# siddC/nbmf_mm

Hardware: AMD Instinct MI355X
Metric: MM-iterations/sec (higher is better)
Workload: dtype f64

## Files before the change

include/nbmf_hip.h:

```cpp
#ifndef NBMF_HIP_H
#define NBMF_HIP_H

#include <stdint.h>

#ifdef __cplusplus
extern "C" {
#endif

#define NBMF_OK 0
#define NBMF_ERR_ARG (-1)
#define NBMF_ERR_HIP (-2)
#define NBMF_ERR_RANGE (-3)
#define NBMF_ERR_STATE (-4)
#define NBMF_ERR_COMM (-5)

#define NBMF_MASK_NONE 0
#define NBMF_MASK_F64 1
#define NBMF_MASK_U8 2

#define NBMF_PROJ_NORMALIZE 0
#define NBMF_PROJ_DUCHI 1

#define NBMF_FLAG_BINARY_PATH 1

// ... 34 lines not shown
#define NBMF_STORAGE_F64_WEIGHTS 2
int nbmf_set_storage(nbmf_ctx* ctx, int storage);

int nbmf_get_n_obs(nbmf_ctx* ctx, double* n_obs);

int nbmf_set_factors(nbmf_ctx* ctx, const double* W_kxm, const double* H_kxn);
int nbmf_get_factors(nbmf_ctx* ctx, double* W_kxm, double* H_kxn);

int nbmf_run(nbmf_ctx* ctx, int max_iter, double tol, double* losses, int* n_iter);

int nbmf_run_batch(nbmf_ctx* ctx, int n_problems, const double* alpha, const double* beta, const double* W0, const double* H0,
                   int max_iter, double tol, double* losses, int* n_iter, double* W_out, double* H_out);
int nbmf_batch_stats(nbmf_ctx* ctx, int* launches, int* problems);
int nbmf_sweep_info(nbmf_ctx* ctx, int* h_chunks, int* h_blocks_per_chunk, int* w_chunks, int* w_blocks_per_chunk);
int nbmf_variant_stats(long long* full_w_launches, long long* ragged_k_launches, long long* loss_assembly_recoveries);

typedef void (*nbmf_progress_fn)(void* user, int first, int count, const double* losses);
int nbmf_set_progress(nbmf_ctx* ctx, nbmf_progress_fn fn, void* user, int every);

int nbmf_small_stats(nbmf_ctx* ctx, int* runs, int* aborted);

int nbmf_engine_stats(long long* persistent_served, long long* persistent_aborted, long long* launches_served);

int nbmf_w_only_steps(nbmf_ctx* ctx, int n_steps);

int nbmf_loss(nbmf_ctx* ctx, double* loss);

int nbmf_loglik(nbmf_ctx* ctx, int clip_theta, double* loglik);

int nbmf_loglik_strict(nbmf_ctx* ctx, double* loglik);
// ... 44 lines not shown
```

nbmf_mm_amd/_hip.py:

```python
from __future__ import annotations

import ctypes
import os
from ctypes import POINTER, byref, c_char_p, c_double, c_int, c_int64, c_void_p

import numpy as np

_HERE = os.path.dirname(os.path.abspath(__file__))

NBMF_OK = 0
NBMF_ERR_ARG = -1
NBMF_ERR_HIP = -2
NBMF_ERR_RANGE = -3
NBMF_ERR_STATE = -4
NBMF_ERR_COMM = -5

MASK_NONE, MASK_F64, MASK_U8 = 0, 1, 2
PROJ_NORMALIZE, PROJ_DUCHI = 0, 1
FLAG_BINARY_PATH = 1
STORAGE = {"auto": 0, "f64": 1, "f64w": 2}
MAX_K = 512
PEER_HANDLE_BYTES = 192

SYMBOLS = [
    "nbmf_abi_version", "nbmf_last_error", "nbmf_device_count", "nbmf_create", "nbmf_destroy",
    "nbmf_set_hyper", "nbmf_upload", "nbmf_upload_csr", "nbmf_generate", "nbmf_get_n_obs", "nbmf_set_factors", "nbmf_get_factors",
    "nbmf_run", "nbmf_w_only_steps", "nbmf_loss", "nbmf_loglik", "nbmf_loglik_strict", "nbmf_comm_unique_id", "nbmf_comm_init",
    "nbmf_comm_init_host", "nbmf_peer_export", "nbmf_comm_init_peer", "nbmf_comm_detach",
    "nbmf_timing_enable", "nbmf_timing_get", "nbmf_synchronize", "nbmf_selftest_unary",
    "nbmf_set_progress", "nbmf_device_synchronize", "nbmf_small_stats", "nbmf_generate_slice", "nbmf_set_storage",
    "nbmf_set_exchange_panels", "nbmf_set_peer_timeout_ms", "nbmf_run_batch", "nbmf_batch_stats", "nbmf_sweep_info",
    "nbmf_upload_v", "nbmf_selftest_mfma_peak", "nbmf_engine_stats", "nbmf_source_hash", "nbmf_comm_info", "nbmf_cancel", "nbmf_variant_stats", "nbmf_device_bus_id",
]
DATA_F64, DATA_U8, DATA_F32 = 0, 1, 2


HOST_ALLREDUCE_FN = ctypes.CFUNCTYPE(c_int, c_void_p, POINTER(c_double), c_int64)
PROGRESS_FN = ctypes.CFUNCTYPE(None, c_void_p, c_int, c_int, POINTER(c_double))


class NBMFHipError(RuntimeError):
    """A libnbmf_hip call failed (HIP error, missing GPU, bad state)."""


def library_path() -> str:
    return os.environ.get("NBMF_HIP_LIBRARY", os.path.join(_HERE, "libnbmf_hip.so"))

# ... 70 lines not shown
    lib.nbmf_upload.argtypes = [c_void_p, c_void_p, c_int64, c_int, c_void_p, c_int, c_int64, POINTER(c_int)]
    lib.nbmf_upload_v.argtypes = [c_void_p, c_void_p, c_int, c_int64, c_int, c_void_p, c_int, c_int64, POINTER(c_int)]
    lib.nbmf_selftest_mfma_peak.argtypes = [c_int, c_double, dp, dp, dp]
    lib.nbmf_engine_stats.argtypes = [POINTER(ctypes.c_longlong), POINTER(ctypes.c_longlong), POINTER(ctypes.c_longlong)]
    lib.nbmf_generate.argtypes = [c_void_p, ctypes.c_uint64, c_double, c_double]
    lib.nbmf_generate_slice.argtypes = [c_void_p, ctypes.c_uint64, c_double, c_double, c_int64, c_int64, c_int64]
    lib.nbmf_set_storage.argtypes = [c_void_p, c_int]
    lib.nbmf_get_n_obs.argtypes = [c_void_p, dp]
    lib.nbmf_set_factors.argtypes = [c_void_p, c_void_p, c_void_p]
    lib.nbmf_get_factors.argtypes = [c_void_p, c_void_p, c_void_p]
    lib.nbmf_run.argtypes = [c_void_p, c_int, c_double, c_void_p, POINTER(c_int)]
    lib.nbmf_run_batch.argtypes = [c_void_p, c_int, c_void_p, c_void_p, c_void_p, c_void_p, c_int, c_double, c_void_p, c_void_p,
                                   c_void_p, c_void_p]
    lib.nbmf_batch_stats.argtypes = [c_void_p, POINTER(c_int), POINTER(c_int)]
    lib.nbmf_sweep_info.argtypes = [c_void_p, POINTER(c_int), POINTER(c_int), POINTER(c_int), POINTER(c_int)]
    lib.nbmf_w_only_steps.argtypes = [c_void_p, c_int]
    lib.nbmf_loss.argtypes = [c_void_p, dp]
    lib.nbmf_loglik.argtypes = [c_void_p, c_int, dp]
    lib.nbmf_loglik_strict.argtypes = [c_void_p, dp]
    lib.nbmf_comm_unique_id.argtypes = [c_void_p]
    lib.nbmf_comm_init.argtypes = [c_void_p, c_void_p, c_int, c_int, c_int]
    lib.nbmf_comm_init_host.argtypes = [c_void_p, HOST_ALLREDUCE_FN, c_void_p, c_int, c_int, c_int]
    lib.nbmf_upload_csr.argtypes = [c_void_p, c_void_p, c_void_p, c_int64, c_int, c_void_p, c_void_p, c_int64, POINTER(c_int)]
    lib.nbmf_peer_export.argtypes = [c_void_p, c_int, c_void_p]
    lib.nbmf_comm_init_peer.argtypes = [c_void_p, c_void_p, c_int, c_int, c_int]
    lib.nbmf_comm_detach.argtypes = [c_void_p]
    lib.nbmf_set_exchange_panels.argtypes = [c_void_p, c_int]
    lib.nbmf_set_peer_timeout_ms.argtypes = [c_void_p, c_double]
    lib.nbmf_timing_enable.argtypes = [c_void_p, c_int]
    lib.nbmf_timing_get.argtypes = [c_void_p, dp, POINTER(c_int), dp, POINTER(c_int)]
# ... 181 lines not shown
        ptr = lambda a: a.ctypes.data_as(c_void_p)
        _check(self._lib.nbmf_run_batch(self._h, int(P), ptr(alphas), ptr(betas), ptr(W0), ptr(H0), int(max_iter), float(tol),
                                        ptr(losses), ptr(n_iter), ptr(W), ptr(H)))
        return [losses[p, :n_iter[p]].copy() for p in range(P)], n_iter, W, H

    def batch_stats(self):
        a, b = c_int(0), c_int(0)
        _check(self._lib.nbmf_batch_stats(self._h, byref(a), byref(b)))
        return a.value, b.value

    def sweep_info(self):
        v = [c_int(0) for _ in range(4)]
        _check(self._lib.nbmf_sweep_info(self._h, *[byref(x) for x in v]))
        return dict(zip(("h_chunks", "h_blocks", "w_chunks", "w_blocks"), (x.value for x in v)))

    def w_only_steps(self, n_steps):
        _check(self._lib.nbmf_w_only_steps(self._h, int(n_steps)))

    def loss(self):
        v = c_double(0)
        _check(self._lib.nbmf_loss(self._h, byref(v)))
        return v.value

    def loglik(self, clip_theta=False):
        v = c_double(0)
        _check(self._lib.nbmf_loglik(self._h, int(bool(clip_theta)), byref(v)))
        return v.value

    def loglik_strict(self):
        v = c_double(0)
# ... 136 lines not shown
```

nbmf_mm_amd/csrc/nbmf_hip.hip:

```cpp

#include <hip/hip_runtime.h>
#include <hip/hip_ext.h>

#include <dlfcn.h>
#include <unistd.h>
#include <algorithm>
#include <atomic>
#include <cmath>
#include <cstdarg>
#include <cstdint>
#include <cstdio>
#include <cstdlib>
#include <cstring>
#include <chrono>
#include <condition_variable>
#include <map>
#include <mutex>
#include <string>
#include <type_traits>
#include <vector>

#include "../../include/nbmf_hip.h"

#ifndef NBMF_NO_MFMA
// ... 205 lines not shown
  int data_kind = -1;
  int storage = NBMF_STORAGE_AUTO;
  void *dataA = nullptr, *dataB = nullptr, *maskA = nullptr, *maskB = nullptr;
  unsigned long long *bitsA = nullptr, *bitsB = nullptr;
  double n_obs = 0, n_obs_global = 0;
  double* rowcnt = nullptr;
  double *Wn = nullptr, *WT = nullptr, *WG = nullptr, *Hn = nullptr, *HT = nullptr, *HG = nullptr;
  bool have_factors = false;
  bool padB_ones = false;
  bool w_free = false;
  bool factors_in_range = false;
  int chunksH = 0, CH_H = 0, chunksW = 0, CH_W = 0;
  int *cstartH = nullptr, *cstartW = nullptr;
  double *slabH = nullptr, *slabW = nullptr, *Pbuf = nullptr, *lossbuf = nullptr, *prior = nullptr, *scal = nullptr;
  double* lossfin = nullptr;
  int n_prior_blocks = 0;
  int* flags = nullptr;
  double* losses_d = nullptr;
  int losses_cap = 0;
  double* stage = nullptr;
  size_t stage_bytes = 0;
  unsigned long long* stats = nullptr;
  double alpha = 1.2, beta = 1.2, eps = 1e-8;
  int projection = NBMF_PROJ_NORMALIZE;
  void* comm = nullptr;
  nbmf_host_allreduce_fn host_reduce = nullptr;
  void* host_reduce_user = nullptr;
  double* host_buf = nullptr;
  size_t host_buf_count = 0;
  int nranks = 1, rank = 0;
// ... 413 lines not shown
      if (cnt[w]) fprintf(stderr, " slot %d: %.1f us (%d)", w, dur[w] / cnt[w] * 0.01, cnt[w]);
    fprintf(stderr, "\n");
    std::sort(exits.begin(), exits.end());
    const double us = 0.01;
    fprintf(stderr, "[nbmf] pass<K=%d,data=%d,mode=%d> %zu workgroups: span %.1f us | entries spread over %.1f us | exits: first %.1f, median %.1f, "
                    "last %.1f us before the end | per workgroup: prologue %.2f, loop %.2f, epilogue %.2f us (loss block %.2f, slab stores %.2f) | shader clock in the loops %.3f GHz\n", K, data, mode, live,
            (double)(t_last - t_first) * us, (double)(last_entry - t_first) * us, (double)(t_last - first_exit) * us,
            ((double)t_last - exits[exits.size() / 2]) * us, 0.0, pro / live * us, loop / live * us, epi / live * us, epi_loss / live * us,
            epi_slab / live * us, loop > 0 ? loop_clk / loop * 0.1 : 0.0);
  }
  return hipSuccess;
}

template <int KB, int DATA, int MODE, int TH, bool TINY, bool RAG = false, bool FULL = false>
hipError_t launch_pass_tt(const PassArgs& a_, int chunks, hipStream_t st) {
  if (FULL) g_full_w_launches.fetch_add(1, std::memory_order_relaxed);
  if (RAG) g_ragged_launches.fetch_add(1, std::memory_order_relaxed);
  dim3 grid(a_.Cb / WG_WAVES, chunks);
  constexpr int lds_bytes = pass_lds_bytes(KB, DATA, MODE);
  if (lds_bytes > 65536) {
    hipError_t e = hipFuncSetAttribute((const void*)pass_kernel<KB, DATA, MODE, TH, TINY, RAG, FULL>, hipFuncAttributeMaxDynamicSharedMemorySize, lds_bytes);
    if (e != hipSuccess) return e;
  }
  PassArgs a = a_;
  if (DATA != DATA_BIN && MODE != MODE_W && MODE != MODE_T && pass_log_bits(KB) == 10) {
    hipError_t e = log_table_device(&a.ltab_g);
    if (e != hipSuccess) return e;
  }
  static std::atomic<long> trace_count{0};
  if (MODE != MODE_T && pass_trace_due(trace_count))
// ... 457 lines not shown

int enqueue_h_update_from(nbmf_ctx* c, const double* src, bool slabs, hipStream_t st) {
  const size_t per = (size_t)std::min(c->KP, SLICE_K) * c->nA;
  const int chunks = slabs ? c->chunksH : 1;
  for (int sl = 0; sl < c->KS; ++sl) {
    launch_h_update(c, src + (size_t)sl * chunks * per, chunks, slabs ? per : 0, 0, c->nA, sl, slabs ? pform_inv12(c) : 0.0, st);
    HIPCHK(hipGetLastError());
  }
  c->prior_src = c->prior;
  c->n_prior_src = c->n_prior_blocks;
  return NBMF_OK;
}
int enqueue_h_update(nbmf_ctx* c) { return enqueue_h_update_from(c, c->slabH, true, c->stream); }

template <int GROUPS>
int launch_w_update(nbmf_ctx* c, const double* q, int chunks, double n_div, int projection) {
  const size_t lds_bytes = sizeof(double) * ((size_t)c->KP + 2) * WU_COLS;
  if (lds_bytes > 65536)
    HIPCHK(hipFuncSetAttribute((const void*)w_update_kernel<GROUPS>, hipFuncAttributeMaxDynamicSharedMemorySize, (int)lds_bytes));
  hipLaunchKernelGGL(w_update_kernel<GROUPS>, dim3((unsigned)(c->mA / WU_COLS)), dim3(WU_COLS * GROUPS), lds_bytes, c->stream, q,
                     chunks, c->Wn, c->WT, c->WG, c->k, c->KP, std::min(c->KP, SLICE_K), (long long)c->m, (long long)c->mA, n_div,
                     c->rowcnt, projection, c->flags);
  HIPCHK(hipGetLastError());
  return NBMF_OK;
}
int enqueue_w_update(nbmf_ctx* c, const double* q, int chunks, double n_div, int projection) {
  return c->mA / WU_COLS <= 4LL * c->cus ? launch_w_update<32>(c, q, chunks, n_div, projection)
                                        : launch_w_update<8>(c, q, chunks, n_div, projection);
}

int enqueue_reduce_h_all(nbmf_ctx* c, double* dst, hipStream_t st) {
  const size_t per = (size_t)std::min(c->KP, SLICE_K) * c->nA, tot = (size_t)c->KP * c->nA;
  for (int sl = 0; sl < c->KS; ++sl) {
    launch_reduce_h(c, sl, 0, c->nA, dst + sl * per, c->nA, sl == 0 ? dst + 2 * tot : (double*)nullptr, st);
    HIPCHK(hipGetLastError());
  }
  return NBMF_OK;
}

int enqueue_w_step(nbmf_ctx* c, int projection);

int enqueue_iteration_rows_peer(nbmf_ctx* c, int it, double tol) {
  const size_t per = (size_t)c->KP * c->nA;
  {
    EvScope ev(c, 0, true, c->KS == 1);
    if (c->KS > 1) {
      if (int rc = enqueue_a_sweeps_sliced(c, true, 0, 0)) return rc;
    } else {
      HIPCHK(launch_pass<MODE_H>(c->KB, c->data_kind, h_pass_args(c), c->chunksH, c->stream));
    }
  }
  double* X = c->arena;
  const unsigned long long hs = ++c->hseq;
  const int slots_per_panel = PEER_H_WGS * c->pv.nranks;
  const long long offPR_now = c->offPR + (long long)(hs & 1) * 2 * 2 * PEER_H_WGS * PEER_MAX_RANKS;
// ... 122 lines not shown
  {
    EvScope ev(c, 1);
    HIPCHK(launch_pass<MODE_W>(c->KB, c->data_kind, w, first, s0));
    if (c->npanel == 2) {
      if (two_streams) {
        HIPCHK(hipStreamWaitEvent(s0, c->ev1, 0));
      } else {
        w.chunk0 = first;
        HIPCHK(launch_pass<MODE_W>(c->KB, c->data_kind, w, c->chunksW - first, s0));
      }
    }
  }
  return enqueue_w_update(c, c->slabW, c->chunksW, (double)c->n, c->projection);
}

int enqueue_w_step(nbmf_ctx* c, int projection) {
  if (c->KS > 1) {
    {
      EvScope ev(c, 1);
      if (int rc = enqueue_theta(c, 1)) return rc;
      for (int step = 0; step < c->KS; ++step) {
        const int sl = step == 0 ? c->KS - 1 : step - 1;
        PassArgs w = w_pass_args(c);
        at_slice(c, w, 1, sl);
        w.theta = c->theta;
        if (step == 0)
          HIPCHK((launch_pass_slice<MODE_W, 2>(c->data_kind, w, c->chunksW, c->stream)));
        else
          HIPCHK((launch_pass_slice<MODE_W, 1>(c->data_kind, w, c->chunksW, c->stream)));
      }
    }
    if (is_sharded(c) && c->shard_axis == 1) {
      const long long per = (long long)SLICE_K * c->mA;
      for (int sl = 0; sl < c->KS; ++sl) {
        hipLaunchKernelGGL(reduce_w_kernel, dim3((unsigned)((per + 255) / 256)), dim3(256), 0, c->stream,
                           (const double*)(c->slabW + (size_t)sl * c->chunksW * per), c->Qbuf + sl * per, c->chunksW, per, c->flags);
        HIPCHK(hipGetLastError());
      }
      if (int rc = all_reduce_inplace(c, c->Qbuf, (size_t)c->KP * c->mA)) return rc;
      return enqueue_w_update(c, c->Qbuf, 1, c->n_div_global, projection);
    }
    return enqueue_w_update(c, c->slabW, c->chunksW, (double)c->n, projection);
  }
  PassArgs a = w_pass_args(c);
  {
    EvScope ev(c, 1, true, true);
    HIPCHK(launch_pass<MODE_W>(c->KB, c->data_kind, a, c->chunksW, c->stream));
  }
  const double* q = c->slabW;
  int chunks = c->chunksW;
  double n_div = (double)c->n;
  if (is_sharded(c) && c->shard_axis == 1) {
    const long long per = (long long)c->KP * c->mA;
    hipLaunchKernelGGL(reduce_w_kernel, dim3((unsigned)((per + 255) / 256)), dim3(256), 0, c->stream,
                       (const double*)c->slabW, c->Qbuf, c->chunksW, per, c->flags);
    HIPCHK(hipGetLastError());
    if (int rc = all_reduce_inplace(c, c->Qbuf, (size_t)per)) return rc;
    q = c->Qbuf;
    chunks = 1;
    n_div = c->n_div_global;
  }
  return enqueue_w_update(c, q, chunks, n_div, projection);
}
// ... 556 lines not shown
  for (int** p : {&c->cstartH, &c->cstartW}) {
    if (*p) HIPCHK(dfree(*p));
    *p = nullptr;
  }
  HIPCHK(dmalloc(&c->cstartH, sizeof(int) * bH.size()));
  HIPCHK(dmalloc(&c->cstartW, sizeof(int) * bW.size()));
  HIPCHK(hipMemcpy(c->cstartH, bH.data(), sizeof(int) * bH.size(), hipMemcpyHostToDevice));
  HIPCHK(hipMemcpy(c->cstartW, bW.data(), sizeof(int) * bW.size(), hipMemcpyHostToDevice));
  if (env_set("NBMF_DEBUG"))
    fprintf(stderr, "[nbmf] K_pad=%d path=%d: H-pass %d x %d workgroups (chunk %d blocks, %d slots), W-pass %d x %d (chunk %d, %d slots)\n",
            c->KP, c->data_kind, (int)(c->nA / 64), c->chunksH, c->CH_H, slotsH, (int)(c->mA / 64), c->chunksW, c->CH_W, slotsW);
  for (double** p : {&c->slabH, &c->slabW, &c->lossbuf, &c->lossfin}) {
    if (*p) HIPCHK(dfree(*p));
    *p = nullptr;
  }
  for (unsigned long long** p : {&c->bitsA, &c->bitsB}) {
    if (*p) HIPCHK(dfree(*p));
    *p = nullptr;
  }
  if (c->data_kind == DATA_BIN) {
    const long long n_tiles = (long long)(c->mA / 16) * (c->nA / 16);
    HIPCHK(dmalloc(&c->bitsA, sizeof(unsigned long long) * 8 * (size_t)n_tiles + PASS_SLACK));
    HIPCHK(dmalloc(&c->bitsB, sizeof(unsigned long long) * 8 * (size_t)n_tiles + PASS_SLACK));
    for (int image = 0; image < 2; ++image) {
      hipLaunchKernelGGL(mask_build_kernel, dim3((unsigned)((n_tiles + 3) / 4)), dim3(256), 0, c->stream,
                         (const uint32_t*)(image == 0 ? c->dataA : c->dataB), image == 0 ? c->bitsA : c->bitsB, n_tiles);
      HIPCHK(hipGetLastError());
    }
  }
  const size_t fw = (size_t)c->KP * c->mA * sizeof(double), fh = (size_t)c->KP * c->nA * sizeof(double);
  HIPCHK(dmalloc(&c->slabH, 2 * (size_t)c->chunksH * fh));
  HIPCHK(dmalloc(&c->slabW, (size_t)c->chunksW * fw));
  const size_t n_slots = (size_t)c->chunksH * (c->nA / 16 / WG_WAVES);
  HIPCHK(dmalloc(&c->lossbuf, sizeof(double) * n_slots));
  HIPCHK(dmalloc(&c->lossfin, sizeof(double) * n_slots));
  if (int rc = fill_ll_empty(c)) return rc;
  return NBMF_OK;
}

void comm_release(nbmf_ctx* c, bool recount = false) {
  if (recount && is_sharded(c) && c->shard_axis == 1 && c->data_kind >= 0) {
    hipLaunchKernelGGL(rowcount_kernel, dim3((unsigned)((c->m + 255) / 256)), dim3(256), 0, c->stream, c->dataB, c->maskB,
                       c->data_kind, (long long)(c->nA / 16), (long long)c->m, (long long)c->n, c->rowcnt);
    hipStreamSynchronize(c->stream);
  }
  if (c->comm && g_rccl.CommDestroy) g_rccl.CommDestroy(c->comm);
  c->comm = nullptr;
// ... 155 lines not shown
  ctx_guard.p = nullptr;
  *out = c;
  return NBMF_OK;
}

int nbmf_destroy(nbmf_ctx* c) {
  if (!c) return NBMF_OK;
  hipSetDevice(c->device);
  if (c->stream) hipStreamSynchronize(c->stream);
  comm_release(c);
  if (c->host_buf) hipHostFree(c->host_buf);
  arena_release((ArenaSlot*)c->arena_slot.p);
  void* ptrs[] = {c->dataA, c->dataB, c->maskA, c->maskB, c->rowcnt, c->Wn, c->WT, c->WG, c->Hn, c->HT, c->HG,
                  c->slabH, c->slabW, c->Pbuf, c->lossbuf, c->lossfin, c->prior, c->scal, c->flags, c->losses_d, c->stage, c->stats,
                  c->sbuf, c->Qbuf, c->cstartH, c->cstartW, c->theta, c->small.slab, c->small_batch.slab, c->small_batch.table,
                  c->small_batch.io, c->bitsA, c->bitsB};
  for (void* p : ptrs)
    if (p) dfree(p);
  for (hipEvent_t e : c->ev) hipEventDestroy(e);
  for (hipEvent_t e : {c->evH, c->evF, c->ev1})
    if (e) hipEventDestroy(e);
  if (c->stream2) {
    hipStreamSynchronize(c->stream2);
    hipStreamDestroy(c->stream2);
  }
  if (c->stream) stream_release(c->device, c->stream);
  delete c;
  return NBMF_OK;
}

int nbmf_set_hyper(nbmf_ctx* c, double alpha, double beta, double eps, int projection) {
// ... 379 lines not shown
  const int batch = progress ? c->progress_every : (tol > 0.0) ? 8 : max_iter;
  int reported = 0;
  std::vector<double> fresh;
  auto report = [&](int n_final) -> int {
    if (!progress || n_final <= reported) return NBMF_OK;
    fresh.resize((size_t)(n_final - reported));
    HIPCHK(hipMemcpy(fresh.data(), c->losses_d + reported, sizeof(double) * fresh.size(), hipMemcpyDeviceToHost));
    c->progress(c->progress_user, reported, n_final - reported, fresh.data());
    reported = n_final;
    return NBMF_OK;
  };
  int host_done = 0;
  int it = 0;
  const bool use_graph = env_set("NBMF_USE_GRAPH") && !is_sharded(c) && !c->timing && !progress && max_iter >= 8;
  bool fused_fin = fin_fusable(c) && !use_graph;
  int recoveries = 0;
  int fl[8];
  auto settle = [&](bool at_end, bool* resume) -> int {
    *resume = false;
    HIPCHK(hipMemcpyAsync(fl, c->flags, sizeof fl, hipMemcpyDeviceToHost, c->stream));
    HIPCHK(hipStreamSynchronize(c->stream));
    if (c->timing) timing_collect(c);
    if (int rc = peer_check(c)) return rc;
    if (!fl[6] || !fused_fin || recoveries >= 4 || (at_end && c->cancelled.load(std::memory_order_relaxed))) return NBMF_OK;
    ++recoveries;
    g_loss_assembly_recoveries.fetch_add(1, std::memory_order_relaxed);
    if (env_set("NBMF_DEBUG")) fprintf(stderr, "[nbmf] loss %d could not be assembled inside its sweep within the bound: resuming with separate launches\n", fl[1]);
    fused_fin = false;
    if (int rc = fill_ll_empty(c)) return rc;
    HIPCHK(hipMemsetAsync(c->flags, 0, sizeof(int), c->stream));
    HIPCHK(hipMemsetAsync(c->flags + 6, 0, sizeof(int), c->stream));
    it = fl[1] + 1;
    host_done = 0;
    *resume = true;
    return NBMF_OK;
  };
  hipGraph_t graph = nullptr;
  hipGraphExec_t gexec = nullptr;
// ... 26 lines not shown
          HIPCHK(hipGraphLaunch(gexec, c->stream));
          continue;
        }
        if (is_sharded(c) && c->shard_axis == 0) {
          if (int rc = enqueue_iteration_rows(c, it, tol)) return rc;
          continue;
        }
        if (fused_fin) {
          if (int rc = enqueue_a_sweep(c, true, 0, 0, it - 1, tol)) return rc;
        } else {
          if (int rc = enqueue_a_sweep(c, true)) return rc;
          if (it > 0)
            if (int rc = enqueue_finalize(c, it - 1, tol)) return rc;
        }
        if (int rc = enqueue_h_update(c)) return rc;
        if (int rc = enqueue_w_step(c, c->projection)) return rc;
      }
      if ((tol > 0.0 || progress) && it < max_iter) {
        bool resume = false;
        if (int rc = settle(false, &resume)) return rc;
        if (!resume) {
          host_done = fl[0];
          if (int rc = report(fl[1])) return rc;
        }
      }
      continue;
    }
    if (!host_done) {
      if (fused_fin) {
        if (int rc = enqueue_a_sweep(c, false, 0, 0, max_iter - 1, tol)) return rc;
      } else {
// ... 57 lines not shown

int nbmf_sweep_info(nbmf_ctx* c, int* h_chunks, int* h_blocks, int* w_chunks, int* w_blocks) {
  if (!c) return fail(NBMF_ERR_ARG, "null context");
  if (!c->cstartH) return fail(NBMF_ERR_STATE, "no data on the device yet");
  if (h_chunks) *h_chunks = c->chunksH;
  if (h_blocks) *h_blocks = c->CH_H;
  if (w_chunks) *w_chunks = c->chunksW;
  if (w_blocks) *w_blocks = c->CH_W;
  return NBMF_OK;
}

int nbmf_variant_stats(long long* full_w_launches, long long* ragged_k_launches, long long* loss_assembly_recoveries) {
  if (full_w_launches) *full_w_launches = g_full_w_launches.load(std::memory_order_relaxed);
  if (ragged_k_launches) *ragged_k_launches = g_ragged_launches.load(std::memory_order_relaxed);
  if (loss_assembly_recoveries) *loss_assembly_recoveries = g_loss_assembly_recoveries.load(std::memory_order_relaxed);
  return NBMF_OK;
}

int nbmf_w_only_steps(nbmf_ctx* c, int n_steps) {
  if (int rc = ready(c)) return rc;
  if (n_steps < 0) return fail(NBMF_ERR_ARG, "n_steps must be >= 0");
  if (int rc = set_device(c)) return rc;
  HIPCHK(hipMemsetAsync(c->flags, 0, sizeof(int) * 8, c->stream));
  struct FreeW {
    nbmf_ctx* c;
    ~FreeW() { c->w_free = false; }
  } free_w{c};
  c->w_free = true;
  for (int s = 0; s < n_steps; ++s) {
    if (int rc = enqueue_w_step(c, NBMF_PROJ_NORMALIZE)) return rc;
// ... 449 lines not shown
```

nbmf_mm_amd/csrc/nbmf_pass_kernel.inc:

```

#define NBMF_DIV(y_, d_) ((y_) * rcp_nr(d_))
#define NBMF_DIV2(ya_, da_, yb_, db_, qa_, qb_) \
  {                                             \
    const double it_ = rcp_nr((da_) * (db_));   \
    qa_ = (ya_) * (it_ * (db_));                \
    qb_ = (yb_) * (it_ * (da_));                \
  }

#if NBMF_NO_MFMA
__device__ __forceinline__ d4 mfma_stub(double a, double b, d4 c) {
  __asm__ volatile("" : "+v"(c) : "v"(a), "v"(b));
  return c;
}
#define NBMF_MFMA(a_, b_, c_, x_, y_, z_) mfma_stub((a_), (b_), (c_))
#else
#define NBMF_MFMA(a_, b_, c_, x_, y_, z_) __builtin_amdgcn_mfma_f64_16x16x4f64((a_), (b_), (c_), (x_), (y_), (z_))
#endif

typedef __attribute__((address_space(3))) char lds_char;
typedef const __attribute__((address_space(1))) char glb_char;
typedef const __attribute__((address_space(1))) uint32_t glb_u32;
template <int PPW>
__device__ __forceinline__ void dma_run(glb_char* g, lds_char* l) {
  static_assert(PPW == 2 || PPW == 4, "2 KiB or 4 KiB per wave and image");
// ... 16 lines not shown
struct PassFin {
  int on;
  unsigned long long wait_ticks;
  int t;
  int n_ll, n_prior;
  double ll_pad, am1, bm1, n_obs, tol;
  const double* prior;
  double* losses;
  double* scal;
  int* flags;
};
template <bool SC1>
__device__ __forceinline__ void finalize_block(const double* ll_src, int n_ll, double ll_pad, const double* prior, int n_prior,
                                               double am1, double bm1, double n_obs, double* __restrict__ losses, int t,
                                               double tol, double* __restrict__ scal, int* __restrict__ flags, double (*sh)[4]);

struct PassArgs {
  const void* data;
  const void* mask;
  const double2* ltab_g;
  const double* LT;
  const double* LG;
  const double* RfT;
  double* out1;
  double* out2;
  double* lossbuf;
  const int* done;
  int Rb;
  int Cb;
  const int* chunk_start;
  int chunk0;
  long long C_alloc;
  double eps;
  int strict;
  int clip;
  double* theta;
  int accum;
  int tiny_eps;
  int ksteps, kblocks;
  int full;
  PassFin fin;
  unsigned long long* trace;
};

constexpr int pass_log_bits(int KB) { return KB == 8 ? 8 : 10; }
constexpr int pass_lds_bytes(int KB, int DATA, int MODE) {
  return (KB <= 4 ? STAGE_BYTES : 2 * STAGE_BYTES) + ((DATA != DATA_BIN && MODE != MODE_W && MODE != MODE_T) ? (16 << pass_log_bits(KB)) : 0);
}
constexpr int pass_wgs_per_cu(int KB, int DATA, int MODE) {
  if (KB == 8) return (MODE == MODE_H && DATA != DATA_BIN) ? 1 : 2;
  if (DATA != DATA_BIN && MODE == MODE_H) return 2;
  if (DATA == DATA_F64 && MODE == MODE_L && KB == 1) return 2;
  return 3;
}
template <int KB, int DATA, int MODE, int TH = 0, bool TINY = false, bool RAG = false, bool FULL = false>
__global__ __launch_bounds__(64 * WG_WAVES, pass_wgs_per_cu(KB, DATA, MODE)) void pass_kernel(PassArgs a) {
  static_assert(TH == 0 || MODE != MODE_T, "a Theta sweep does not read Theta");
  static_assert(!FULL || (MODE == MODE_W && DATA == DATA_BIN && TH == 0 && !TINY), "the two-state variant: W sweeps of the binary path's plain variant");
  static_assert(!TINY || MODE != MODE_T, "eps does not change the code of the Theta sweeps");
  static_assert(!RAG || (TH == 0 && !TINY && MODE != MODE_T && KB <= 4), "the ragged-K variant: one slice, plain variant, fused sweeps, up to the K = 64 layout");
  [[maybe_unused]] const int ksteps = a.ksteps, kblocks = a.kblocks;
  constexpr bool PRODUCTS = (MODE == MODE_H || MODE == MODE_W);
  constexpr int K = 16 * KB;
  constexpr int S = K / 4;
  constexpr int NB = (KB >= 4) ? 1 : 4 / KB;
  constexpr int BLK = K * 16;
  constexpr int STAGE_D = 2 * NB * BLK;
  constexpr int N2 = NB * BLK / 2;
  extern __shared__ __attribute__((aligned(16))) double lds[];
// ... 628 lines not shown
        __hip_atomic_store(a.lossbuf + (size_t)chunk * gridDim.x + bx, t, __ATOMIC_RELAXED, __HIP_MEMORY_SCOPE_AGENT);
    }
  }

  [[maybe_unused]] unsigned long long tr3 = 0, tr4 = 0;
  if (a.trace) tr3 = wall_clock64();
  const int q = lane >> 4, c = lane & 15;
  {
    if (MODE == MODE_W) {
      s2 += __shfl_xor(s2, 16, 64);
      s2 += __shfl_xor(s2, 32, 64);
    }
    [[maybe_unused]] const double inv12 = 1.0 / c12;
    double* o1 = a.out1 + (size_t)chunk * K * a.C_alloc + (size_t)cb * 16 + c;
    double* o2 = (MODE == MODE_H) ? a.out2 + (size_t)chunk * K * a.C_alloc + (size_t)cb * 16 + c : nullptr;
    if (PRODUCTS) {
#pragma unroll
      for (int kb = 0; kb < KB; ++kb) {
#pragma unroll
        for (int r = 0; r < 4; ++r) {
          const size_t k = 16 * kb + 4 * r + q;
          if (MODE == MODE_H) {
            o1[k * a.C_alloc] = acc1[kb][r];
            o2[k * a.C_alloc] = acc2[kb][r];
          } else {
            o1[k * a.C_alloc] = ZE_W ? __builtin_fma(s2, inv12, acc1[kb][r]) : acc1[kb][r] + s2;
          }
        }
      }
    }
// ... 58 lines not shown
```

nbmf_mm_amd/csrc/nbmf_update_kernels.inc:

```

__device__ __forceinline__ size_t t_index(long long k, long long x, int KS, long long lenA) {
  return (size_t)(k / KS) * KS * lenA + (size_t)((x >> 4) * KS + (k % KS)) * 16 + (x & 15);
}
__device__ __forceinline__ size_t g_index(long long k, long long x, int KS, long long lenA) {
  const long long kk = k % KS;
  return (size_t)(k / KS) * KS * lenA + (size_t)(x >> 4) * KS * 16 + (kk >> 4) * 256 + (x & 15) * 16 + (kk & 15);
}

__device__ __forceinline__ double ordered_sum256(const double* __restrict__ p, int n, int stride, double* sh4) {
  double s = 0.0;
  for (int j = threadIdx.x; j < n; j += 256) s += p[(size_t)j * stride];
  s = wave_sum(s);
  __syncthreads();
  if ((threadIdx.x & 63) == 0) sh4[threadIdx.x >> 6] = s;
  __syncthreads();
  return ((sh4[0] + sh4[1]) + sh4[2]) + sh4[3];
}

__global__ __launch_bounds__(256) void reduce_h_kernel(const double* __restrict__ slab1, const double* __restrict__ slab2,
                                                       int chunks, long long per , long long nA,
                                                       long long c0, long long wp, long long dst_ld, int KP,
                                                       double* __restrict__ dst1, double* __restrict__ dst2,
                                                       const double* __restrict__ lossbuf,
                                                       int n_loss, double ll_pad, double* __restrict__ ll_dst,
// ... 177 lines not shown
  if (flags[0]) return;
  if (t < 0) {
    const int armed = flags[3];
    __syncthreads();
    if (!armed) {
      if (threadIdx.x == 0) flags[3] = 1;
      return;
    }
    t = flags[2];
  }
  __shared__ double sh[3][4];
  finalize_block<false>(ll_src, n_ll, ll_pad, prior, n_prior, am1, bm1, n_obs, losses, t, tol, scal, flags, sh);
}

constexpr int WU_COLS = 32;
template <int WU_GROUPS>
__global__ __launch_bounds__(WU_COLS * WU_GROUPS) void w_update_kernel(const double* __restrict__ slab, int chunks, double* __restrict__ Wn,
                                                       double* __restrict__ WT, double* __restrict__ WG, int K, int KP,
                                                       int KS , long long m,
                                                       long long mA, double n_div,
                                                       const double* __restrict__ rowcnt, int projection,
                                                       const int* done) {
  extern __shared__ __attribute__((aligned(16))) double tile[];
  if (*done) return;
  const int c = threadIdx.x & (WU_COLS - 1), g = threadIdx.x / WU_COLS;
  const long long i = (long long)blockIdx.x * WU_COLS + c;
  const size_t per = (size_t)KS * mA;
  const bool live = i < m;
  double div = n_div;
  if (live && projection == NBMF_PROJ_DUCHI && rowcnt) div = fmax(rowcnt[i], 1.0);
  for (int k = g; k < K; k += WU_GROUPS) {
    double w = 0.0;
    if (live) {
      double qv = 0.0;
      const double* sk = slab + (size_t)(k / KS) * chunks * per + (size_t)(k % KS) * mA + i;
      for (int ch = 0; ch < chunks; ++ch) qv += sk[(size_t)ch * per];
      w = (Wn[(size_t)k * mA + i] * qv) / div;
    }
    tile[k * WU_COLS + c] = w;
  }
  __syncthreads();
  double* par = tile + (size_t)KP * WU_COLS;
  if (g == 0) {
    double sum = 0.0;
    for (int k = 0; k < K; ++k) sum += tile[k * WU_COLS + c];
    double tau = 0.0, scale = 1.0;
    if (projection == NBMF_PROJ_DUCHI) {
      tau = (sum - 1.0) / K;
      int cnt = K;
      for (int it = 0; it < K; ++it) {
        double s = 0.0;
        int c2 = 0;
        for (int k = 0; k < K; ++k) {
          const double v = tile[k * WU_COLS + c];
          if (v > tau) {
            s += v;
            ++c2;
          }
        }
        if (c2 == 0) break;
        const bool same = (c2 == cnt);
        tau = (s - 1.0) / c2;
        cnt = c2;
        if (same) break;
      }
    } else {
      scale = sum;
    }
    par[c] = scale;
    par[WU_COLS + c] = tau;
  }
  __syncthreads();
  const double scale = par[c], tau = par[WU_COLS + c];
  for (int k = g; k < KP; k += WU_GROUPS) {
    double w = 0.0;
    if (live && k < K) {
      const double v = tile[k * WU_COLS + c];
      w = (projection == NBMF_PROJ_DUCHI) ? fmax(v - tau, 0.0) : v / scale;
    }
    Wn[(size_t)k * mA + i] = w;
    WT[t_index(k, i, KS, mA)] = w;
    WG[g_index(k, i, KS, mA)] = w;
  }
}

__global__ void set_factor_kernel(const double* __restrict__ src, double* __restrict__ Fn, double* __restrict__ FT,
                                  double* __restrict__ FG, int K, int KP, int KS, long long len, long long lenA) {
  const long long idx = (long long)blockIdx.x * blockDim.x + threadIdx.x;
  if (idx >= (long long)KP * lenA) return;
  const long long k = idx / lenA, x = idx % lenA;
  const double v = (k < K && x < len) ? src[k * len + x] : 0.0;
  Fn[idx] = v;
  FT[t_index(k, x, KS, lenA)] = v;
  FG[g_index(k, x, KS, lenA)] = v;
}

__global__ void factor_range_kernel(const double* __restrict__ Wn, const double* __restrict__ Hn, int K, long long m,
// ... 29 lines not shown
```

Baseline: 202.8.

## Fuse W update into W pass epilogue with cross-chunk ticket handoff

When the W sweep has at most two chunks and no sharding, the pass kernel's epilogue now applies the multiplicative W update and projection directly. It uses an atomic ticket so the second chunk's workgroup waits for the first chunk's partial sums through the slab. This removes the separate w_update_kernel launch and its slab re-read per iteration. A bounded spin with a timeout flag falls back to separate launches, and the host resumes from the failing iteration. The cost is extra epilogue work, atomic handoff, and slab reset traffic.

After: 201.6. About the same (-0.6%).

```diff
diff --git a/include/nbmf_hip.h b/include/nbmf_hip.h
--- a/include/nbmf_hip.h
+++ b/include/nbmf_hip.h
@@ -72,6 +72,7 @@
 int nbmf_batch_stats(nbmf_ctx* ctx, int* launches, int* problems);
 int nbmf_sweep_info(nbmf_ctx* ctx, int* h_chunks, int* h_blocks_per_chunk, int* w_chunks, int* w_blocks_per_chunk);
 int nbmf_variant_stats(long long* full_w_launches, long long* ragged_k_launches, long long* loss_assembly_recoveries);
+int nbmf_fused_w_stats(nbmf_ctx* ctx, long long* fused_sweeps, long long* recoveries);
 
 typedef void (*nbmf_progress_fn)(void* user, int first, int count, const double* losses);
 int nbmf_set_progress(nbmf_ctx* ctx, nbmf_progress_fn fn, void* user, int every);
diff --git a/nbmf_mm_amd/_hip.py b/nbmf_mm_amd/_hip.py
--- a/nbmf_mm_amd/_hip.py
+++ b/nbmf_mm_amd/_hip.py
@@ -31,6 +31,7 @@
     "nbmf_set_progress", "nbmf_device_synchronize", "nbmf_small_stats", "nbmf_generate_slice", "nbmf_set_storage",
     "nbmf_set_exchange_panels", "nbmf_set_peer_timeout_ms", "nbmf_run_batch", "nbmf_batch_stats", "nbmf_sweep_info",
     "nbmf_upload_v", "nbmf_selftest_mfma_peak", "nbmf_engine_stats", "nbmf_source_hash", "nbmf_comm_info", "nbmf_cancel", "nbmf_variant_stats", "nbmf_device_bus_id",
+    "nbmf_fused_w_stats",
 ]
 DATA_F64, DATA_U8, DATA_F32 = 0, 1, 2
 
@@ -131,6 +132,7 @@
                                    c_void_p, c_void_p]
     lib.nbmf_batch_stats.argtypes = [c_void_p, POINTER(c_int), POINTER(c_int)]
     lib.nbmf_sweep_info.argtypes = [c_void_p, POINTER(c_int), POINTER(c_int), POINTER(c_int), POINTER(c_int)]
+    lib.nbmf_fused_w_stats.argtypes = [c_void_p, POINTER(ctypes.c_longlong), POINTER(ctypes.c_longlong)]
     lib.nbmf_w_only_steps.argtypes = [c_void_p, c_int]
     lib.nbmf_loss.argtypes = [c_void_p, dp]
     lib.nbmf_loglik.argtypes = [c_void_p, c_int, dp]
@@ -342,6 +344,11 @@
         _check(self._lib.nbmf_sweep_info(self._h, *[byref(x) for x in v]))
         return dict(zip(("h_chunks", "h_blocks", "w_chunks", "w_blocks"), (x.value for x in v)))
 
+    def fused_w_stats(self):
+        a, b = ctypes.c_longlong(0), ctypes.c_longlong(0)
+        _check(self._lib.nbmf_fused_w_stats(self._h, byref(a), byref(b)))
+        return a.value, b.value
+
     def w_only_steps(self, n_steps):
         _check(self._lib.nbmf_w_only_steps(self._h, int(n_steps)))
 
diff --git a/nbmf_mm_amd/csrc/nbmf_hip.hip b/nbmf_mm_amd/csrc/nbmf_hip.hip
--- a/nbmf_mm_amd/csrc/nbmf_hip.hip
+++ b/nbmf_mm_amd/csrc/nbmf_hip.hip
@@ -243,6 +243,8 @@
   int *cstartH = nullptr, *cstartW = nullptr;
   double *slabH = nullptr, *slabW = nullptr, *Pbuf = nullptr, *lossbuf = nullptr, *prior = nullptr, *scal = nullptr;
   double* lossfin = nullptr;
+  int* wfuse = nullptr;
+  long long fused_w_sweeps = 0, fused_w_recoveries = 0;
   int n_prior_blocks = 0;
   int* flags = nullptr;
   double* losses_d = nullptr;
@@ -686,6 +688,7 @@
 
 template <int KB, int DATA, int MODE, int TH, bool TINY, bool RAG = false, bool FULL = false>
 hipError_t launch_pass_tt(const PassArgs& a_, int chunks, hipStream_t st) {
+  if (a_.wup.on && !pass_has_wup(KB, MODE, TH, RAG)) return hipErrorInvalidValue;
   if (FULL) g_full_w_launches.fetch_add(1, std::memory_order_relaxed);
   if (RAG) g_ragged_launches.fetch_add(1, std::memory_order_relaxed);
   dim3 grid(a_.Cb / WG_WAVES, chunks);
@@ -1173,19 +1176,19 @@
 int enqueue_h_update(nbmf_ctx* c) { return enqueue_h_update_from(c, c->slabH, true, c->stream); }
 
 template <int GROUPS>
-int launch_w_update(nbmf_ctx* c, const double* q, int chunks, double n_div, int projection) {
+int launch_w_update(nbmf_ctx* c, const double* q, int chunks, double n_div, int projection, const int* applied, int epoch) {
   const size_t lds_bytes = sizeof(double) * ((size_t)c->KP + 2) * WU_COLS;
   if (lds_bytes > 65536)
     HIPCHK(hipFuncSetAttribute((const void*)w_update_kernel<GROUPS>, hipFuncAttributeMaxDynamicSharedMemorySize, (int)lds_bytes));
   hipLaunchKernelGGL(w_update_kernel<GROUPS>, dim3((unsigned)(c->mA / WU_COLS)), dim3(WU_COLS * GROUPS), lds_bytes, c->stream, q,
                      chunks, c->Wn, c->WT, c->WG, c->k, c->KP, std::min(c->KP, SLICE_K), (long long)c->m, (long long)c->mA, n_div,
-                     c->rowcnt, projection, c->flags);
+                     c->rowcnt, projection, c->flags, applied, epoch);
   HIPCHK(hipGetLastError());
   return NBMF_OK;
 }
-int enqueue_w_update(nbmf_ctx* c, const double* q, int chunks, double n_div, int projection) {
-  return c->mA / WU_COLS <= 4LL * c->cus ? launch_w_update<32>(c, q, chunks, n_div, projection)
-                                        : launch_w_update<8>(c, q, chunks, n_div, projection);
+int enqueue_w_update(nbmf_ctx* c, const double* q, int chunks, double n_div, int projection, const int* applied = nullptr, int epoch = 0) {
+  return c->mA / WU_COLS <= 4LL * c->cus ? launch_w_update<32>(c, q, chunks, n_div, projection, applied, epoch)
+                                        : launch_w_update<8>(c, q, chunks, n_div, projection, applied, epoch);
 }
 
 int enqueue_reduce_h_all(nbmf_ctx* c, double* dst, hipStream_t st) {
@@ -1197,7 +1200,7 @@
   return NBMF_OK;
 }
 
-int enqueue_w_step(nbmf_ctx* c, int projection);
+int enqueue_w_step(nbmf_ctx* c, int projection, int fuse_epoch = 0, int rest_of_epoch = 0);
 
 int enqueue_iteration_rows_peer(nbmf_ctx* c, int it, double tol) {
   const size_t per = (size_t)c->KP * c->nA;
@@ -1350,7 +1353,23 @@
   return enqueue_w_update(c, c->slabW, c->chunksW, (double)c->n, c->projection);
 }
 
-int enqueue_w_step(nbmf_ctx* c, int projection) {
+bool w_update_fusable(const nbmf_ctx* c) {
+  if (c->KB >= 4 && c->k < 16 * c->KB) return false;
+  if (c->mA >= (1LL << 26)) return false;
+  return !is_sharded(c) && c->KS == 1 && c->chunksW <= 2 && c->wfuse && !env_set("NBMF_NO_FUSED_W_UPDATE");
+}
+int* w_applied(const nbmf_ctx* c) { return c->wfuse + c->mA / 64; }
+int w_fuse_arm(nbmf_ctx* c) {
+  HIPCHK(hipMemsetAsync(c->wfuse, 0, sizeof(int) * (size_t)(c->mA / 64 + c->mA / 16), c->stream));
+  if (c->chunksW == 2) {
+    const size_t n = (size_t)c->chunksW * c->KP * c->mA;
+    hipLaunchKernelGGL(fill_u64_kernel, dim3((unsigned)((n + 255) / 256)), dim3(256), 0, c->stream, (unsigned long long*)c->slabW, n, LL_EMPTY);
+    HIPCHK(hipGetLastError());
+  }
+  return NBMF_OK;
+}
+
+int enqueue_w_step(nbmf_ctx* c, int projection, int fuse_epoch, int rest_of_epoch) {
   if (c->KS > 1) {
     {
       EvScope ev(c, 1);
@@ -1379,10 +1398,29 @@
     return enqueue_w_update(c, c->slabW, c->chunksW, (double)c->n, projection);
   }
   PassArgs a = w_pass_args(c);
+  if (fuse_epoch > 0) {
+    a.wup.on = 1;
+    a.wup.epoch = fuse_epoch;
+    a.wup.wait_ticks = env_int("NBMF_FUSED_W_FAULT", 0) == 2 ? 0ull : LL_WAIT_TICKS;
+    a.wup.projection = projection;
+    a.wup.K = c->k;
+    a.wup.m = c->m;
+    a.wup.n_div = (double)c->n;
+    a.wup.rowcnt = c->rowcnt;
+    a.wup.Wn = c->Wn;
+    a.wup.WT = c->WT;
+    a.wup.WG = c->WG;
+    a.wup.ticket = (unsigned*)c->wfuse;
+    a.wup.applied = w_applied(c);
+    a.wup.flags = c->flags;
+    ++c->fused_w_sweeps;
+  }
   {
     EvScope ev(c, 1, true, true);
     HIPCHK(launch_pass<MODE_W>(c->KB, c->data_kind, a, c->chunksW, c->stream));
   }
+  if (fuse_epoch > 0) return NBMF_OK;
+  if (rest_of_epoch > 0) return enqueue_w_update(c, c->slabW, c->chunksW, (double)c->n, projection, w_applied(c), rest_of_epoch);
   const double* q = c->slabW;
   int chunks = c->chunksW;
   double n_div = (double)c->n;
@@ -1969,6 +2007,8 @@
     if (*p) HIPCHK(dfree(*p));
     *p = nullptr;
   }
+  if (c->wfuse) HIPCHK(dfree(c->wfuse));
+  c->wfuse = nullptr;
   for (unsigned long long** p : {&c->bitsA, &c->bitsB}) {
     if (*p) HIPCHK(dfree(*p));
     *p = nullptr;
@@ -1986,6 +2026,7 @@
   const size_t fw = (size_t)c->KP * c->mA * sizeof(double), fh = (size_t)c->KP * c->nA * sizeof(double);
   HIPCHK(dmalloc(&c->slabH, 2 * (size_t)c->chunksH * fh));
   HIPCHK(dmalloc(&c->slabW, (size_t)c->chunksW * fw));
+  HIPCHK(dmalloc(&c->wfuse, sizeof(int) * (size_t)(c->mA / 64 + c->mA / 16)));
   const size_t n_slots = (size_t)c->chunksH * (c->nA / 16 / WG_WAVES);
   HIPCHK(dmalloc(&c->lossbuf, sizeof(double) * n_slots));
   HIPCHK(dmalloc(&c->lossfin, sizeof(double) * n_slots));
@@ -2171,7 +2212,7 @@
   void* ptrs[] = {c->dataA, c->dataB, c->maskA, c->maskB, c->rowcnt, c->Wn, c->WT, c->WG, c->Hn, c->HT, c->HG,
                   c->slabH, c->slabW, c->Pbuf, c->lossbuf, c->lossfin, c->prior, c->scal, c->flags, c->losses_d, c->stage, c->stats,
                   c->sbuf, c->Qbuf, c->cstartH, c->cstartW, c->theta, c->small.slab, c->small_batch.slab, c->small_batch.table,
-                  c->small_batch.io, c->bitsA, c->bitsB};
+                  c->small_batch.io, c->bitsA, c->bitsB, c->wfuse};
   for (void* p : ptrs)
     if (p) dfree(p);
   for (hipEvent_t e : c->ev) hipEventDestroy(e);
@@ -2581,6 +2622,9 @@
   int it = 0;
   const bool use_graph = env_set("NBMF_USE_GRAPH") && !is_sharded(c) && !c->timing && !progress && max_iter >= 8;
   bool fused_fin = fin_fusable(c) && !use_graph;
+  bool fused_w = w_update_fusable(c) && !use_graph;
+  if (fused_w)
+    if (int rc = w_fuse_arm(c)) return rc;
   int recoveries = 0;
   int fl[8];
   auto settle = [&](bool at_end, bool* resume) -> int {
@@ -2589,6 +2633,18 @@
     HIPCHK(hipStreamSynchronize(c->stream));
     if (c->timing) timing_collect(c);
     if (int rc = peer_check(c)) return rc;
+    if (fl[7] && fused_w && !(at_end && c->cancelled.load(std::memory_order_relaxed))) {
+      ++c->fused_w_recoveries;
+      if (env_set("NBMF_DEBUG")) fprintf(stderr, "[nbmf] the W sweep of iteration %d could not apply all of its update within the bound: resuming with separate launches\n", fl[7] - 1);
+      fused_w = false;
+      HIPCHK(hipMemsetAsync(c->flags, 0, sizeof(int), c->stream));
+      HIPCHK(hipMemsetAsync(c->flags + 7, 0, sizeof(int), c->stream));
+      if (int rc = enqueue_w_step(c, c->projection, 0, fl[7])) return rc;
+      it = fl[7];
+      host_done = 0;
+      *resume = true;
+      return NBMF_OK;
+    }
     if (!fl[6] || !fused_fin || recoveries >= 4 || (at_end && c->cancelled.load(std::memory_order_relaxed))) return NBMF_OK;
     ++recoveries;
     g_loss_assembly_recoveries.fetch_add(1, std::memory_order_relaxed);
@@ -2645,7 +2701,7 @@
             if (int rc = enqueue_finalize(c, it - 1, tol)) return rc;
         }
         if (int rc = enqueue_h_update(c)) return rc;
-        if (int rc = enqueue_w_step(c, c->projection)) return rc;
+        if (int rc = enqueue_w_step(c, c->projection, fused_w ? it + 1 : 0)) return rc;
       }
       if ((tol > 0.0 || progress) && it < max_iter) {
         bool resume = false;
@@ -2733,6 +2789,13 @@
   if (full_w_launches) *full_w_launches = g_full_w_launches.load(std::memory_order_relaxed);
   if (ragged_k_launches) *ragged_k_launches = g_ragged_launches.load(std::memory_order_relaxed);
   if (loss_assembly_recoveries) *loss_assembly_recoveries = g_loss_assembly_recoveries.load(std::memory_order_relaxed);
+  return NBMF_OK;
+}
+
+int nbmf_fused_w_stats(nbmf_ctx* c, long long* fused_sweeps, long long* recoveries) {
+  if (!c) return fail(NBMF_ERR_ARG, "null context");
+  if (fused_sweeps) *fused_sweeps = c->fused_w_sweeps;
+  if (recoveries) *recoveries = c->fused_w_recoveries;
   return NBMF_OK;
 }
 
diff --git a/nbmf_mm_amd/csrc/nbmf_pass_kernel.inc b/nbmf_mm_amd/csrc/nbmf_pass_kernel.inc
--- a/nbmf_mm_amd/csrc/nbmf_pass_kernel.inc
+++ b/nbmf_mm_amd/csrc/nbmf_pass_kernel.inc
@@ -54,6 +54,29 @@
 __device__ __forceinline__ void finalize_block(const double* ll_src, int n_ll, double ll_pad, const double* prior, int n_prior,
                                                double am1, double bm1, double n_obs, double* __restrict__ losses, int t,
                                                double tol, double* __restrict__ scal, int* __restrict__ flags, double (*sh)[4]);
+
+struct PassWup {
+  int on;
+  int epoch;
+  unsigned long long wait_ticks;
+  int projection, K;
+  long long m;
+  double n_div;
+  const double* rowcnt;
+  double *Wn, *WT, *WG;
+  unsigned* ticket;
+  int* applied;
+  int* flags;
+};
+__device__ __forceinline__ size_t t_index(long long k, long long x, int KS, long long lenA);
+__device__ __forceinline__ size_t g_index(long long k, long long x, int KS, long long lenA);
+__device__ __forceinline__ double wu_div(bool live, long long i, double n_div, const double* __restrict__ rowcnt, int projection);
+__device__ __forceinline__ double wu_times(double w, double qv);
+__device__ __forceinline__ double wu_over(double p, double div);
+__device__ __forceinline__ void wu_column(const double* tile, int stride, int K, int projection, double* scale_out, double* tau_out);
+__device__ __forceinline__ double wu_value(double v, double scale, double tau, int projection);
+__device__ __forceinline__ void wu_store(double* __restrict__ Wn, double* __restrict__ WT, double* __restrict__ WG, long long k,
+                                         long long i, int KS, long long mA, double w);
 
 struct PassArgs {
   const void* data;
@@ -80,6 +103,7 @@
   int ksteps, kblocks;
   int full;
   PassFin fin;
+  PassWup wup;
   unsigned long long* trace;
 };
 
@@ -93,6 +117,7 @@
   if (DATA == DATA_F64 && MODE == MODE_L && KB == 1) return 2;
   return 3;
 }
+constexpr bool pass_has_wup(int KB, int MODE, int TH, bool RAG) { return MODE == MODE_W && TH == 0 && !(RAG && KB >= 4); }
 template <int KB, int DATA, int MODE, int TH = 0, bool TINY = false, bool RAG = false, bool FULL = false>
 __global__ __launch_bounds__(64 * WG_WAVES, pass_wgs_per_cu(KB, DATA, MODE)) void pass_kernel(PassArgs a) {
   static_assert(TH == 0 || MODE != MODE_T, "a Theta sweep does not read Theta");
@@ -751,6 +776,111 @@
     [[maybe_unused]] const double inv12 = 1.0 / c12;
     double* o1 = a.out1 + (size_t)chunk * K * a.C_alloc + (size_t)cb * 16 + c;
     double* o2 = (MODE == MODE_H) ? a.out2 + (size_t)chunk * K * a.C_alloc + (size_t)cb * 16 + c : nullptr;
+    constexpr bool WUP = pass_has_wup(KB, MODE, TH, RAG);
+    if (WUP && a.wup.on) {
+      const unsigned long long rowB = (unsigned long long)a.C_alloc * 8ull;
+      unsigned lane_slab = (unsigned)q * (unsigned)rowB + (unsigned)c * 8u;
+      typedef __attribute__((address_space(1))) char glb_wchar;
+      typedef __attribute__((address_space(1))) unsigned long long glb_u64;
+#pragma unroll
+      for (int kb = 0; kb < KB; ++kb) {
+#pragma unroll
+        for (int r = 0; r < 4; ++r) acc1[kb][r] = 0.0 + (ZE_W ? __builtin_fma(s2, inv12, acc1[kb][r]) : acc1[kb][r] + s2);
+      }
+      bool apply = true;
+      if (gridDim.y == 2) {
+        volatile unsigned* tk = (volatile unsigned*)lds;
+        if (threadIdx.x == 0) *tk = __hip_atomic_fetch_add(a.wup.ticket + bx, 1u, __ATOMIC_RELAXED, __HIP_MEMORY_SCOPE_AGENT);
+        __syncthreads();
+        const bool second = __builtin_amdgcn_readfirstlane((int)(*tk & 1u)) != 0;
+        __syncthreads();
+        const int sc = second ? (chunk ^ 1) : chunk;
+        const unsigned long long sb = scalar64((unsigned long long)(a.out1 + (size_t)sc * K * a.C_alloc + (size_t)cb * 16));
+        if (!second) {
+#pragma unroll
+          for (int kb = 0; kb < KB; ++kb) {
+#pragma unroll
+            for (int r = 0; r < 4; ++r)
+              __hip_atomic_store((glb_u64*)((glb_wchar*)(sb + (unsigned long long)(16 * kb + 4 * r) * rowB) + lane_slab),
+                                 (unsigned long long)__double_as_longlong(acc1[kb][r]), __ATOMIC_RELAXED, __HIP_MEMORY_SCOPE_AGENT);
+          }
+          apply = false;
+        } else {
+          constexpr int GK = KB < 4 ? KB : 4;
+          const unsigned long long t0 = (unsigned long long)wall_clock64();
+#pragma unroll
+          for (int g0 = 0; g0 < KB; g0 += GK) {
+            d4 oth[GK];
+            for (;;) {
+              bool missing = false;
+              __asm__ volatile("" : "+v"(lane_slab));
+#pragma unroll
+              for (int kb = 0; kb < GK; ++kb) {
+#pragma unroll
+                for (int r = 0; r < 4; ++r) {
+                  const unsigned long long v = __hip_atomic_load((glb_u64*)((glb_wchar*)(sb + (unsigned long long)(16 * (g0 + kb) + 4 * r) * rowB) + lane_slab),
+                                                                 __ATOMIC_RELAXED, __HIP_MEMORY_SCOPE_AGENT);
+                  missing |= v == LL_EMPTY;
+                  oth[kb][r] = __longlong_as_double((long long)v);
+                }
+              }
+              if (__builtin_amdgcn_ballot_w64(missing) == 0ull) break;
+              if ((unsigned long long)wall_clock64() - t0 > a.wup.wait_ticks) {
+                apply = false;
+                break;
+              }
+              __builtin_amdgcn_s_sleep(8);
+            }
+            if (!apply) break;
+#pragma unroll
+            for (int kb = 0; kb < GK; ++kb) {
+#pragma unroll
+              for (int r = 0; r < 4; ++r) {
+                __hip_atomic_store((glb_u64*)((glb_wchar*)(sb + (unsigned long long)(16 * (g0 + kb) + 4 * r) * rowB) + lane_slab), LL_EMPTY,
+                                   __ATOMIC_RELAXED, __HIP_MEMORY_SCOPE_AGENT);
+                acc1[g0 + kb][r] = (chunk == 0) ? acc1[g0 + kb][r] + oth[kb][r] : (0.0 + oth[kb][r]) + acc1[g0 + kb][r];
+              }
+            }
+          }
+          if (!apply && lane == 0) {
+            a.wup.flags[0] = 1;
+            a.wup.flags[7] = a.wup.epoch;
+          }
+        }
+      }
+      if (apply) {
+        const long long i = (long long)cb * 16 + c;
+        const bool live = i < a.wup.m;
+        const int projection = a.wup.projection, Kr = a.wup.K;
+        const double div = wu_div(live, i, a.wup.n_div, a.wup.rowcnt, projection);
+        double* tile = lds + wave * (K * 16) + c;
+#pragma unroll
+        for (int kb = 0; kb < KB; ++kb) {
+#pragma unroll
+          for (int r = 0; r < 4; ++r) tile[(16 * kb + 4 * r + q) * 16] = acc1[kb][r];
+        }
+        {
+          double w[S];
+#pragma unroll
+          for (int s = 0; s < S; ++s) w[s] = a.RfT[((size_t)cb * S + s) * 64 + lane];
+#pragma unroll
+          for (int s = 0; s < S; ++s) tile[(4 * s + q) * 16] = wu_times(w[s], tile[(4 * s + q) * 16]);
+        }
+#pragma unroll 1
+        for (int k = q; k < K; k += 4) tile[k * 16] = live ? wu_over(tile[k * 16], div) : 0.0;
+        __builtin_amdgcn_fence(__ATOMIC_RELEASE, "wavefront");
+        __builtin_amdgcn_wave_barrier();
+        __builtin_amdgcn_fence(__ATOMIC_ACQUIRE, "wavefront");
+        double scale, tau;
+        wu_column(tile, 16, Kr, projection, &scale, &tau);
+#pragma unroll 1
+        for (int k = q; k < K; k += 4) {
+          const double w = (live && k < Kr) ? wu_value(tile[k * 16], scale, tau, projection) : 0.0;
+          wu_store(a.wup.Wn, a.wup.WT, a.wup.WG, k, i, K, a.C_alloc, w);
+        }
+        if (lane == 0) a.wup.applied[cb] = a.wup.epoch;
+      }
+    } else
     if (PRODUCTS) {
 #pragma unroll
       for (int kb = 0; kb < KB; ++kb) {
diff --git a/nbmf_mm_amd/csrc/nbmf_update_kernels.inc b/nbmf_mm_amd/csrc/nbmf_update_kernels.inc
--- a/nbmf_mm_amd/csrc/nbmf_update_kernels.inc
+++ b/nbmf_mm_amd/csrc/nbmf_update_kernels.inc
@@ -215,73 +215,88 @@
 }
 
 constexpr int WU_COLS = 32;
+__device__ __forceinline__ double wu_div(bool live, long long i, double n_div, const double* __restrict__ rowcnt, int projection) {
+  double div = n_div;
+  if (live && projection == NBMF_PROJ_DUCHI && rowcnt) div = fmax(rowcnt[i], 1.0);
+  return div;
+}
+__device__ __forceinline__ double wu_times(double w, double qv) { return w * qv; }
+__device__ __forceinline__ double wu_over(double p, double div) { return p / div; }
+__device__ __forceinline__ double wu_product(double w, double qv, double div) { return wu_over(wu_times(w, qv), div); }
+__device__ __forceinline__ void wu_column(const double* tile, int stride, int K, int projection, double* scale_out, double* tau_out) {
+  double sum = 0.0;
+  for (int k = 0; k < K; ++k) sum += tile[k * stride];
+  double tau = 0.0, scale = 1.0;
+  if (projection == NBMF_PROJ_DUCHI) {
+    tau = (sum - 1.0) / K;
+    int cnt = K;
+    for (int it = 0; it < K; ++it) {
+      double s = 0.0;
+      int c2 = 0;
+      for (int k = 0; k < K; ++k) {
+        const double v = tile[k * stride];
+        if (v > tau) {
+          s += v;
+          ++c2;
+        }
+      }
+      if (c2 == 0) break;
+      const bool same = (c2 == cnt);
+      tau = (s - 1.0) / c2;
+      cnt = c2;
+      if (same) break;
+    }
+  } else {
+    scale = sum;
+  }
+  *scale_out = scale;
+  *tau_out = tau;
+}
+__device__ __forceinline__ double wu_value(double v, double scale, double tau, int projection) {
+  return (projection == NBMF_PROJ_DUCHI) ? fmax(v - tau, 0.0) : v / scale;
+}
+__device__ __forceinline__ void wu_store(double* __restrict__ Wn, double* __restrict__ WT, double* __restrict__ WG, long long k,
+                                         long long i, int KS, long long mA, double w) {
+  Wn[(size_t)k * mA + i] = w;
+  WT[t_index(k, i, KS, mA)] = w;
+  WG[g_index(k, i, KS, mA)] = w;
+}
+
 template <int WU_GROUPS>
 __global__ __launch_bounds__(WU_COLS * WU_GROUPS) void w_update_kernel(const double* __restrict__ slab, int chunks, double* __restrict__ Wn,
                                                        double* __restrict__ WT, double* __restrict__ WG, int K, int KP,
                                                        int KS , long long m,
                                                        long long mA, double n_div,
                                                        const double* __restrict__ rowcnt, int projection,
-                                                       const int* done) {
+                                                       const int* done, const int* __restrict__ applied, int epoch) {
   extern __shared__ __attribute__((aligned(16))) double tile[];
   if (*done) return;
   const int c = threadIdx.x & (WU_COLS - 1), g = threadIdx.x / WU_COLS;
   const long long i = (long long)blockIdx.x * WU_COLS + c;
   const size_t per = (size_t)KS * mA;
   const bool live = i < m;
-  double div = n_div;
-  if (live && projection == NBMF_PROJ_DUCHI && rowcnt) div = fmax(rowcnt[i], 1.0);
+  const bool skip = applied && applied[i >> 4] == epoch;
+  const double div = wu_div(live, i, n_div, rowcnt, projection);
   for (int k = g; k < K; k += WU_GROUPS) {
     double w = 0.0;
-    if (live) {
+    if (live && !skip) {
       double qv = 0.0;
       const double* sk = slab + (size_t)(k / KS) * chunks * per + (size_t)(k % KS) * mA + i;
       for (int ch = 0; ch < chunks; ++ch) qv += sk[(size_t)ch * per];
-      w = (Wn[(size_t)k * mA + i] * qv) / div;
+      w = wu_product(Wn[(size_t)k * mA + i], qv, div);
     }
     tile[k * WU_COLS + c] = w;
   }
   __syncthreads();
   double* par = tile + (size_t)KP * WU_COLS;
-  if (g == 0) {
-    double sum = 0.0;
-    for (int k = 0; k < K; ++k) sum += tile[k * WU_COLS + c];
-    double tau = 0.0, scale = 1.0;
-    if (projection == NBMF_PROJ_DUCHI) {
-      tau = (sum - 1.0) / K;
-      int cnt = K;
-      for (int it = 0; it < K; ++it) {
-        double s = 0.0;
-        int c2 = 0;
-        for (int k = 0; k < K; ++k) {
-          const double v = tile[k * WU_COLS + c];
-          if (v > tau) {
-            s += v;
-            ++c2;
-          }
-        }
-        if (c2 == 0) break;
-        const bool same = (c2 == cnt);
-        tau = (s - 1.0) / c2;
-        cnt = c2;
-        if (same) break;
-      }
-    } else {
-      scale = sum;
-    }
-    par[c] = scale;
-    par[WU_COLS + c] = tau;
-  }
+  if (g == 0) wu_column(tile + c, WU_COLS, K, projection, par + c, par + WU_COLS + c);
   __syncthreads();
   const double scale = par[c], tau = par[WU_COLS + c];
+  if (skip) return;
   for (int k = g; k < KP; k += WU_GROUPS) {
     double w = 0.0;
-    if (live && k < K) {
-      const double v = tile[k * WU_COLS + c];
-      w = (projection == NBMF_PROJ_DUCHI) ? fmax(v - tau, 0.0) : v / scale;
-    }
-    Wn[(size_t)k * mA + i] = w;
-    WT[t_index(k, i, KS, mA)] = w;
-    WG[g_index(k, i, KS, mA)] = w;
+    if (live && k < K) w = wu_value(tile[k * WU_COLS + c], scale, tau, projection);
+    wu_store(Wn, WT, WG, k, i, KS, mA, w);
   }
 }
 
```
